# aiforvision/OCTA-autosegmentation

Measured on AMD Instinct MI355X. Metric: synthetic OCTA samples/sec (graph + 304x304 image + 1216x1216 label triples), higher is better.
Workload: dtype f64

## Files before the change

include/octa_hip.h:

```cpp
#ifndef OCTA_HIP_H
#define OCTA_HIP_H

#include <stddef.h>
#include <stdint.h>

#ifdef __cplusplus
extern "C" {
#endif

typedef struct octa_ctx octa_ctx;


int octa_abi_version(void);

const char *octa_last_error(void);

int octa_ctx_create(int device, octa_ctx **out);
void octa_ctx_destroy(octa_ctx *ctx);

size_t octa_ctx_scratch_bytes(const octa_ctx *ctx);

int octa_rasterize_2d(octa_ctx *ctx, int B, const double *d_edges, const int64_t *h_edge_off,
                      const uint8_t *d_keep, int no_pixels_x, int no_pixels_y, int mip_axis,
                      double min_radius, double max_radius, uint8_t *d_out, void *stream);
// ... 284 lines not shown
int octa_sim_geometry(int num_cus, int *h_out4);

int octa_sim_is_large(const octa_sim *sim);

int octa_sim_fields(octa_sim *sim, int sample, double *h_oxy, int64_t cap_oxy, int64_t *n_oxy, double *h_co2,
                    int64_t cap_co2, int64_t *n_co2);

int octa_sim_kat_kd_order(octa_ctx *ctx, const double *h_pts, int64_t n, const uint8_t *h_need, int32_t *h_indices);

int octa_sim_kat_kd_order_signflag(octa_ctx *ctx, const double *h_pts, int64_t n, const uint8_t *h_need, int32_t need_bits, int32_t *h_indices);

int octa_sim_kat_sample(octa_ctx *ctx, const double *h_cand, int64_t n_cand, const double *h_npos, const double *h_nrad, int64_t n_art,
                        double *h_oxy, int64_t n_oxy, int64_t cap_oxy, double eps_n, double eps_k, double eps_s, const double *h_cst8,
                        int64_t *h_n_out);

#ifdef __cplusplus
}
#endif
#endif
```

octa_autosegmentation_amd/_native.py:

```python
import contextlib
import ctypes
import os
import random as _random
import threading

import numpy as np

HERE = os.path.dirname(os.path.abspath(__file__))
LIB_PATH = os.environ.get("OCTA_HIP_LIB") or os.path.join(HERE, "liboctahip.so")

_lib = None
_ctxs = {}
_lock = threading.Lock()

c_void_p, c_int, c_double, c_size_t = ctypes.c_void_p, ctypes.c_int, ctypes.c_double, ctypes.c_size_t


def _struct(name, ints, ptrs):
    fields = [("struct_size", ctypes.c_uint32)] + [(k, c_int) for k in ints.split()] + [("slope", ctypes.c_float)] + [(k, c_void_p) for k in ptrs.split()]
    return type(name, (ctypes.Structure,), {"_fields_": fields})


Conv3x3Args = _struct("Conv3x3Args", "N H W Cin Cout stride in_dilation tap_mask out_scale out_off_y out_off_x C1 CY1 nslot",
                      "d_x d_x2 d_w d_y d_y2 d_scale1 d_shift1 d_scale2 d_shift2 d_stat_partials d_stat_slots d_residual")
# ... 113 lines not shown
    "octa_headn_nhwc_bwd": (c_int, [c_void_p, c_void_p, c_void_p, c_void_p, c_int, ctypes.c_int64, c_int, c_int, c_void_p, c_void_p, c_void_p, c_void_p]),
    "octa_conv3x3_c1_fwd": (c_int, [c_void_p, c_void_p, c_void_p, c_void_p, c_int, c_int, c_int, c_int, c_void_p, c_int, c_void_p]),
    "octa_fft2_c2c_f64_workspace_bytes": (c_size_t, [c_int, c_int, c_int]),
    "octa_fft2_c2c_f64": (c_int, [c_void_p, c_void_p, c_int, c_int, c_int, c_int, c_void_p, c_void_p]),
    "octa_oof_workspace_bytes": (c_size_t, [c_int, c_int, c_int]),
    "octa_oof_2d": (c_int, [c_void_p, c_void_p, c_int, c_int, c_int, c_void_p, c_void_p]),
    "octa_oof_2d_response": (c_int, [c_void_p, c_void_p, c_int, c_int, c_int, c_void_p, c_void_p]),
    "octa_frangi_workspace_bytes": (c_size_t, [c_int, c_int, c_int, c_int]),
    "octa_frangi_2d": (c_int, [c_void_p, c_void_p, c_int, c_int, c_int, c_int, c_void_p, c_void_p, ctypes.c_float, c_double, c_double, c_int, c_void_p, c_void_p]),
    "octa_frangi_hessian": (c_int, [c_void_p, c_void_p, c_void_p, c_void_p, c_int, c_int, c_int, c_int, c_void_p, ctypes.c_float, c_int, c_void_p, c_void_p]),
    "octa_frangi_eigenvalues": (c_int, [c_void_p, c_void_p, c_void_p, c_void_p, c_int, c_int, c_int, c_int, c_void_p, ctypes.c_float, c_int, c_void_p, c_void_p]),
    "octa_sim_kat_kd_order": (c_int, [c_void_p, c_void_p, ctypes.c_int64, c_void_p, c_void_p]),
    "octa_sim_kat_kd_order_signflag": (c_int, [c_void_p, c_void_p, ctypes.c_int64, c_void_p, ctypes.c_int32, c_void_p]),
    "octa_sim_kat_sample": (c_int, [c_void_p, c_void_p, ctypes.c_int64, c_void_p, c_void_p, ctypes.c_int64, c_void_p, ctypes.c_int64, ctypes.c_int64,
                                    c_double, c_double, c_double, c_void_p, c_void_p]),
}


class OctaHipError(RuntimeError):
    pass


def lib():
    global _lib
    if _lib is None:
        with _lock:
            if _lib is None:
                if not os.path.exists(LIB_PATH):
                    raise OctaHipError(
                        f"{LIB_PATH} is missing: build it with `python -m octa_autosegmentation_amd.build` "
# ... 113 lines not shown
```

octa_autosegmentation_amd/csrc/sim.hip:

```cpp

#include <chrono>
#include <vector>

#include "common.h"
#include "sim_host.h"
#include <thread>
#include <atomic>
#include <cstdlib>
#include <cstring>

using namespace OCTA_SIMK;

#if OCTA_SIM_LARGE
#define OCTA_SIM_T octa_simL_impl
#define OCTA_SIM_FN(name) octa_simL_##name
#else
#define OCTA_SIM_T octa_simS_impl
#define OCTA_SIM_FN(name) octa_simS_##name
#endif
#define octa_sim_create OCTA_SIM_FN(create)
#define octa_sim_destroy OCTA_SIM_FN(destroy)
#define octa_sim_run OCTA_SIM_FN(run)
#define octa_sim_run_states OCTA_SIM_FN(run_states)
#define octa_sim_np_state OCTA_SIM_FN(np_state)
#define octa_sim_edge_offsets OCTA_SIM_FN(edge_offsets)
#define octa_sim_export_edges OCTA_SIM_FN(export_edges)
#define octa_sim_export_edges_device OCTA_SIM_FN(export_edges_device)
#define octa_sim_trace OCTA_SIM_FN(trace)
#define octa_sim_stats OCTA_SIM_FN(stats)
#define octa_sim_kd_paths OCTA_SIM_FN(kd_paths)
#define octa_sim_assign_paths OCTA_SIM_FN(assign_paths)
#define octa_sim_fields OCTA_SIM_FN(fields)
#define octa_sim_service_stats OCTA_SIM_FN(service_stats)
#define octa_sim_geometry OCTA_SIM_FN(geometry)
#define octa_sim_spans OCTA_SIM_FN(spans)
#define octa_sim_timing OCTA_SIM_FN(timing)
#define octa_sim_kat_kd_order OCTA_SIM_FN(kat_kd_order)
#define octa_sim_kat_kd_order_signflag OCTA_SIM_FN(kat_kd_order_signflag)
#define octa_sim_kat_sample OCTA_SIM_FN(kat_sample)
struct OCTA_SIM_T;
extern "C" void octa_sim_destroy(OCTA_SIM_T *S);
extern "C" long long octa_sim_next_ticket(void);
extern "C" int *octa_sim_launch_flag(int device);

namespace {

constexpr int SIM_THREADS = SIM_THREADS_PER_WG;
constexpr int SIM_WG_PER_CU = 2;
#if OCTA_SIM_LARGE
constexpr size_t SIM_LDS = 2048;
#else
constexpr size_t SIM_LDS = SIM_LDS_BYTES;
static_assert((size_t)KD_MAILBOX_OFF + KD_MAILBOX_BYTES <= (size_t)SIM_USER_BYTES && SIM_WG_PER_CU * SIM_LDS <= 160 * 1024, "LDS budget");
#endif
// ... 1360 lines not shown
        ok(hipFuncSetAttribute(reinterpret_cast<const void *>(sim_kat_sample_kernel), hipFuncAttributeMaxDynamicSharedMemorySize, (int)SIM_LDS), "attribute")) {
        hipLaunchKernelGGL(sim_kat_sample_kernel, dim3(1), dim3(SIM_THREADS), SIM_LDS, 0, A, C, P);
        if (ok(hipGetLastError(), "launch") && ok(hipMemcpy(&sc, A.sc, sizeof(sc), hipMemcpyDeviceToHost), "result")) {
            if (sc.err) { octa::set_error("octa_sim_kat_sample: the phase set error bits %d", sc.err); rc = -3; }
            else {
                *h_n_out = sc.n_oxy;
                const int64_t n = sc.n_oxy < cap_oxy ? sc.n_oxy : cap_oxy;
                if (n) ok(hipMemcpy(h_oxy, A.oxy, sizeof(double) * 3 * n, hipMemcpyDeviceToHost), "sinks back");
            }
        }
    }
    (void)hipFree(d);
    return rc;
}

#endif

extern "C" int octa_sim_service_stats(OCTA_SIM_T *S, double *h_out4) {
    if (!S || !S->ran || !h_out4) { octa::set_error("octa_sim_service_stats: run the simulation first"); return -2; }
    h_out4[0] = (double)S->diag_tickets; h_out4[1] = S->diag_max_gap_ms; h_out4[2] = (double)S->diag_relaunches; h_out4[3] = (double)S->diag_parked;
    h_out4[4] = S->diag_max_bif_ms;
    return 0;
}

extern "C" int octa_sim_geometry(int num_cus, int *h_out4) {
    if (!h_out4) { octa::set_error("octa_sim_geometry: null output"); return -2; }
    h_out4[0] = SIM_THREADS; h_out4[1] = SIM_WG_PER_CU; h_out4[2] = (int)SIM_LDS; h_out4[3] = SIM_WG_PER_CU * (num_cus > 0 ? num_cus : 256);
    return 0;
}

// ... 13 lines not shown
```

octa_autosegmentation_amd/csrc/sim_api.cpp:

```cpp
#include <cstdlib>
#include <cstring>
#include <new>

#include "common.h"

extern "C" {
struct octa_simS_impl;
struct octa_simL_impl;
#define OCTA_DECL(SFX, T)                                                                                                                       \
    int octa_sim##SFX##_create(octa_ctx *, const octa_sim_config *, int, T **);                                                                 \
    void octa_sim##SFX##_destroy(T *);                                                                                                          \
    int octa_sim##SFX##_run(T *, const uint32_t *, const uint64_t *, octa_bif_fn, void *, void *);                                              \
    int octa_sim##SFX##_run_states(T *, const double *, const double *, const uint32_t *, const uint32_t *, octa_bif_fn, void *, void *);       \
    int octa_sim##SFX##_np_state(T *, int, uint32_t *);                                                                                         \
    int octa_sim##SFX##_edge_offsets(T *, int64_t *, int64_t *);                                                                                \
    int octa_sim##SFX##_export_edges(T *, double *);                                                                                            \
    int octa_sim##SFX##_export_edges_device(T *, double *, void *);                                                                             \
    int octa_sim##SFX##_trace(T *, int32_t *);                                                                                                  \
    int octa_sim##SFX##_stats(T *, int64_t *);                                                                                                  \
    int octa_sim##SFX##_kd_paths(T *, int64_t *);                                                                                               \
    int octa_sim##SFX##_assign_paths(T *, int64_t *);                                                                                           \
    int octa_sim##SFX##_spans(T *, int64_t *);                                                                                                  \
    int octa_sim##SFX##_timing(T *, double *);                                                                                                  \
    int octa_sim##SFX##_service_stats(T *, double *);                                                                                           \
    int octa_sim##SFX##_geometry(int, int *);                                                                                                   \
    int octa_sim##SFX##_fields(T *, int, double *, int64_t, int64_t *, double *, int64_t, int64_t *);
OCTA_DECL(S, octa_simS_impl)
OCTA_DECL(L, octa_simL_impl)
#undef OCTA_DECL
int octa_simS_kat_kd_order(octa_ctx *, const double *, int64_t, const uint8_t *, int32_t *);
int octa_simS_kat_kd_order_signflag(octa_ctx *, const double *, int64_t, const uint8_t *, int32_t, int32_t *);
int octa_simS_kat_sample(octa_ctx *, const double *, int64_t, const double *, const double *, int64_t, double *, int64_t, int64_t, double, double, double,
                         const double *, int64_t *);
}

#include <atomic>
#include <mutex>
static std::atomic<long long> g_sim_launches{0};
extern "C" long long octa_sim_next_ticket(void) { return g_sim_launches.fetch_add(1, std::memory_order_acq_rel) + 1; }
extern "C" long long octa_sim_launch_count(void) { return g_sim_launches.load(std::memory_order_acquire); }
extern "C" int *octa_sim_launch_flag(int device) {
    static std::mutex m;
    static int *flags[64] = {};
    if (device < 0 || device >= 64) return nullptr;
    std::lock_guard<std::mutex> g(m);
    if (!flags[device]) {
        int prev = 0;
        if (hipGetDevice(&prev) != hipSuccess || hipSetDevice(device) != hipSuccess) return nullptr;
// ... 62 lines not shown
extern "C" int octa_sim_kd_paths(octa_sim *sim, int64_t *t) { NEED(sim, "octa_sim_kd_paths") return FWD(octa_simS_kd_paths(sim->s, t), octa_simL_kd_paths(sim->l, t)); }
extern "C" int octa_sim_assign_paths(octa_sim *sim, int64_t *t) { NEED(sim, "octa_sim_assign_paths") return FWD(octa_simS_assign_paths(sim->s, t), octa_simL_assign_paths(sim->l, t)); }
extern "C" int octa_sim_spans(octa_sim *sim, int64_t *t) { NEED(sim, "octa_sim_spans") return FWD(octa_simS_spans(sim->s, t), octa_simL_spans(sim->l, t)); }
extern "C" int octa_sim_timing(octa_sim *sim, double *t) { NEED(sim, "octa_sim_timing") return FWD(octa_simS_timing(sim->s, t), octa_simL_timing(sim->l, t)); }
extern "C" int octa_sim_service_stats(octa_sim *sim, double *t) { NEED(sim, "octa_sim_service_stats") return FWD(octa_simS_service_stats(sim->s, t), octa_simL_service_stats(sim->l, t)); }
extern "C" int octa_sim_fields(octa_sim *sim, int k, double *o, int64_t co, int64_t *no, double *c, int64_t cc, int64_t *nc) {
    NEED(sim, "octa_sim_fields") return FWD(octa_simS_fields(sim->s, k, o, co, no, c, cc, nc), octa_simL_fields(sim->l, k, o, co, no, c, cc, nc));
}
extern "C" int octa_sim_geometry(int num_cus, int *h_out4) { return octa_simS_geometry(num_cus, h_out4); }
extern "C" int octa_sim_kat_kd_order(octa_ctx *ctx, const double *p, int64_t n, const uint8_t *need, int32_t *o) { return octa_simS_kat_kd_order(ctx, p, n, need, o); }
extern "C" int octa_sim_kat_kd_order_signflag(octa_ctx *ctx, const double *p, int64_t n, const uint8_t *need, int32_t bits, int32_t *o) { return octa_simS_kat_kd_order_signflag(ctx, p, n, need, bits, o); }
extern "C" int octa_sim_kat_sample(octa_ctx *ctx, const double *cand, int64_t n_cand, const double *npos, const double *nrad, int64_t n_art, double *oxy,
                                   int64_t n_oxy, int64_t cap_oxy, double eps_n, double eps_k, double eps_s, const double *cst8, int64_t *n_out) {
    return octa_simS_kat_sample(ctx, cand, n_cand, npos, nrad, n_art, oxy, n_oxy, cap_oxy, eps_n, eps_k, eps_s, cst8, n_out);
}
extern "C" int octa_sim_is_large(const octa_sim *sim) { return sim && sim->large ? 1 : 0; }
```

octa_autosegmentation_amd/csrc/sim_core.h:

```cpp
#pragma once
#include <cmath>
#include <cstdint>
#include <cstring>
#include <algorithm>
#include "gpow.h"
#include "glibc_trig.h"

#ifndef OCTA_SIM_LARGE
#define OCTA_SIM_LARGE 0
#endif
#if OCTA_SIM_LARGE
#define OCTA_SIMK octa_simk_large
#else
#define OCTA_SIMK octa_simk
#endif
namespace OCTA_SIMK {

#if OCTA_SIM_LARGE
typedef unsigned int idx_t;
typedef unsigned long long kdw_t;
constexpr int IDX_BITS = 18;
constexpr int GROUP_BITS = 17;
constexpr int NCAP = 1 << 17;
constexpr int OCAP = 1 << 18;
// ... 919 lines not shown
#if defined(__HIP_DEVICE_COMPILE__)
    atomicMin(p, v);
#else
    if (v < *p) *p = v;
#endif
}

constexpr int KD_TAB_OFF = OCAP * (int)sizeof(kdw_t);
constexpr int KD_BOX_BYTES = KD_RANGES * 24;
static_assert(KD_RANGES >= OCAP / 17 + 1, "ranges per level");
static_assert(KD_MAILBOX_OFF % 16 == 0 && KD_MAILBOX_OFF >= KD_TAB_OFF + KD_RANGES * KD_TAB_BYTES_PER_RANGE, "kd tables overlap the mailbox");
static_assert(KD_MAILBOX_OFF + (KD_BOX_BYTES > KD_MAILBOX_BYTES ? KD_BOX_BYTES : KD_MAILBOX_BYTES) <= SIM_USER_BYTES, "kd table layout (box table and mailbox share their area)");
OCTA_HD inline void kd_build(const Blk &b, const double *pts, int n, idx_t *out_idx, idx_t *out_rank,
                              float *xy, double zlo, double zhi, long *kdprof = nullptr, const unsigned char *need = nullptr,
                              const bool flag_in_sign = false, const unsigned char need_bits = 0xff) {
#if defined(__HIP_DEVICE_COMPILE__) && !defined(OCTA_SIM_PROF_ASSIGN) && !defined(OCTA_SIM_PROF_SAMPLE) && !defined(OCTA_SIM_PROF_SET) && !defined(OCTA_SIM_PROF_MAIL) && !defined(OCTA_SIM_PROF_SEQ) && !defined(OCTA_SIM_PROF_SEQ2)
#define KDP(slot) do { if (kdprof && b.tid == 0) { long _t = (long)wall_clock64(); kdprof[slot] += _t - _kt; _kt = _t; } } while (0)
    long _kt = (long)wall_clock64();
#else
#define KDP(slot) do { } while (0)
#endif
    kdw_t *kv = reinterpret_cast<kdw_t *>(b.user_of<1>());
    idx_t *tab = reinterpret_cast<idx_t *>(b.user_of<1>() + KD_TAB_OFF);
    idx_t *rs = tab, *re = tab + KD_RANGES;
    idx_t *rs2 = tab + 2 * KD_RANGES, *re2 = tab + 3 * KD_RANGES;
    signed char *rd = reinterpret_cast<signed char *>(tab + 4 * KD_RANGES);
    unsigned *bbf = reinterpret_cast<unsigned *>(b.user_of<1>() + KD_MAILBOX_OFF);
#if defined(__HIP_DEVICE_COMPILE__) && !OCTA_SIM_LARGE
    if ((size_t)n * (sizeof(kdw_t) + 8) + 8 <= (size_t)KD_TAB_OFF)
        xy = reinterpret_cast<float *>(b.user_of<1>() + (((size_t)n * sizeof(kdw_t) + 7) & ~(size_t)7));
#endif
// ... 1165 lines not shown
#else
#ifndef OCTA_SIM_SAMPLE_GRID
#define OCTA_SIM_SAMPLE_GRID 96
#endif
#ifndef OCTA_SIM_SAMPLE_NODE_FIRST
#define OCTA_SIM_SAMPLE_NODE_FIRST 0
#endif
constexpr int SMP_CH = 2048;
constexpr int SMP_GRID = OCTA_SIM_SAMPLE_GRID;
constexpr int SMP_GP_MAX = 1024, SMP_GPAIR_CAP = 2048;
constexpr size_t SMP_OFF_LIVE = (size_t)SMP_CH * 24, SMP_OFF_PP = SMP_OFF_LIVE + SMP_CH, SMP_OFF_SLOT = SMP_OFF_PP + (size_t)SMP_GP_MAX * 24;
static_assert(SMP_CH < 0xffff && SMP_GRID * SMP_GRID < 0xffff, "slots and cells are 16-bit, 0xffff marks a candidate that is not valid");
static_assert(SMP_OFF_PP + ((size_t)SMP_GRID * SMP_GRID + 2) / 2 * 4 <= SMP_OFF_SLOT && SMP_OFF_SLOT + (size_t)SMP_CH * 2 <= (size_t)SIM_USER_BYTES, "candidate grid layout");
static_assert((size_t)SMP_GP_MAX * 7 + (size_t)SMP_GPAIR_CAP * 2 <= SMP_OFF_LIVE && (size_t)ACCCAP * 24 <= SMP_OFF_PP + (size_t)SMP_GP_MAX * 24, "greedy acceptance tables");
#if defined(OCTA_SIM_SAMPLE_COUNT) && !defined(__HIP_DEVICE_COMPILE__)
static long smp_count[12];
static int smp_count_pass = 5;
#define SMP_COUNT(i, v) (smp_count[i] += (v))
#else
#define SMP_COUNT(i, v) ((void)0)
#endif
struct SmpGrid {
    int nc;
    double x0, inv;
    unsigned *endw;
    const double *pos;
    unsigned char *live;
};
OCTA_HD inline int smp_cell1(const SmpGrid &G, double x) { return grid_clampi((int)floor((x - G.x0) * G.inv), G.nc - 1); }
OCTA_HD inline int smp_end(const SmpGrid &G, int c) { return (int)((G.endw[c >> 1] >> ((c & 1) * 16)) & 0xffffu); }
template <class F>
// ... 1184 lines not shown
        sc->new_begin[f] = n_before;
        sc->new_end[f] = n_nodes;
        sc->n_nodes[f] = n_nodes;
        sc->py_pos = py_pos;
        if (b.tid == 0) {
            if (err) sc->err |= err;
            sc->murray_steps += steps + n_def;
            sc->murray_deferred += n_def;
#if defined(__HIP_DEVICE_COMPILE__)
            b.coll()[91] = n_def <= MURRAY_FLUSH_LDS ? 0 : n_def;
#else
            b.coll()[91] = n_def;
#endif
            sc->n_bif += n_bif;
            sc->respec += respec;
            sc->kdprof[7] += t_acc[0]; (void)t_acc[1]; (void)t_acc[2];
#if defined(OCTA_SIM_PROF_SEQ2) && defined(__HIP_DEVICE_COMPILE__)
            q2[3] = t_acc[1];
            for (int k = 0; k < 7; k++) sc->kdprof[k] += q2[k];
#endif
#if defined(OCTA_SIM_PROF_SEQ) && defined(__HIP_DEVICE_COMPILE__)
            sc->kdprof[1] += (long)wall_clock64() - _q1; sc->kdprof[2] += t_acc[0]; sc->kdprof[4] += t_acc[2]; sc->kdprof[5] += t_acc[3]; sc->kdprof[6] += n_def;
#endif
        }
#if defined(__HIP_DEVICE_COMPILE__)
        if (n_def > 0 && n_def <= MURRAY_FLUSH_LDS) {
            const long tp0 = (long)wall_clock64();
            for (int base = 0; base < n_def; base += MURRAY_FLUSH_WAVE)
                murray_flush_prepare_wave(A, f, L, n_def, A.fl_rec + (size_t)f * MURRAY_FLUSH_LDS, base);
            if (b.tid == 0) { sc->fl_pending[f] = n_def; sc->kdprof[7] += (long)wall_clock64() - tp0; }
        }
#endif
    }
#if defined(__HIP_DEVICE_COMPILE__)
    else {
        static_assert(SIM_THREADS_PER_WG == 256, "the ordered pass hands its side work to waves 1 - 3");
        const int wv = b.tid >> 6;
        if (wv == 1) side(side_lds);
        const int nw = (f == 1 || pend_other > 2 * MURRAY_FLUSH_WAVE) ? 3 : 2;
        const int w = wv == 2 ? 0 : (wv == 3 ? 1 : 2);
        if (w < nw && w * 64 < pend_other) {
            const int rounds = murray_flush_rounds_wave(A.nrad_of(1 - f), L.log_tab, L.exp_tab, L.fl_val, L.fl_done, A.fl_rec + (size_t)(1 - f) * MURRAY_FLUSH_LDS,
                                                        pend_other, w, nw, true);
            if (b.tid == 128) sc->flush_rounds += rounds;
        }
// ... 2 lines not shown
    (void)side; (void)side_lds;
#endif
#undef SEQT
#undef SEQ2_TOP
#undef SEQ2_SEL
#undef SEQ2_END
#undef SEQ2_ARG
    b.sync();
#if defined(__HIP_DEVICE_COMPILE__)
    if (b.tid == 0 && pend_other > 0) sc->fl_pending[1 - f] = 0;
#endif
    {
        long t0 = OCTA_FLUSH_T0();
        const int rounds = murray_flush(b, A, f, L, b.coll()[91]);
        if (b.tid == 0) {
            sc->kdprof[7] += OCTA_FLUSH_T0() - t0; sc->flush_rounds += rounds;
#if defined(OCTA_SIM_PROF_SEQ) && defined(__HIP_DEVICE_COMPILE__)
            sc->kdprof[3] += OCTA_FLUSH_T0() - t0;
#endif
        }
    }
    b.sync();
}

OCTA_HD inline void murray_flush_pending(const Blk &b, const SimArrays &A) {
#if defined(__HIP_DEVICE_COMPILE__)
    b.sync();
    double *fl_val = reinterpret_cast<double *>(b.user_of<8>());
    int *fl_done = reinterpret_cast<int *>(fl_val + MURRAY_FLUSH_LDS);
    for (int f = 0; f < 2; f++) {
        const int n = OCTA_UNI(A.sc->fl_pending[f]);
// ... 93 lines not shown
    (void)A; (void)f; (void)n;
    return false;
#else
    return OCTA_UNI((int)(A.nn_prev_of(f) != nullptr && A.sc->n_cached[f] == n)) != 0;
#endif
}

#if defined(__HIP_DEVICE_COMPILE__)
#define OCTA_SUBPROF(sc, slot, t0) do { if (b.tid == 0) { long _t1 = (long)wall_clock64(); (sc)->prof[slot] += _t1 - (t0); (t0) = _t1; } } while (0)
#define OCTA_SUBPROF_T0() ((long)wall_clock64())
#else
#define OCTA_SUBPROF(sc, slot, t0) do { (void)(t0); } while (0)
#define OCTA_SUBPROF_T0() 0L
#endif

OCTA_HD inline void phase_satisfy_art(const Blk &b, const SimArrays &A, const SimConst &C, const IterParams &P) {
    const double zext = C.sz;
    SampleScalars *sc = A.sc;
    const int nb = sc->new_begin[0], ne = sc->new_end[0];
    const int n_new = ne - nb, n_oxy = sc->n_oxy;
    if (n_new <= 0 || n_oxy <= 0) return;
    const double ek = P.eps_k, ek2 = ek * ek;
    long t0 = OCTA_SUBPROF_T0();
    for (int i = b.tid; i < n_oxy; i += b.nth) A.removed[i] = 0;
    int *ctl = b.coll() + 100;
    if (b.tid == 0) { ctl[0] = 0; ctl[1] = 0; ctl[2] = 0; }
    unsigned char *xf = reinterpret_cast<unsigned char *>(A.nn);
    static_assert((size_t)NCAP <= (size_t)OCAP * sizeof(int), "group flags fit the nearest-node list");
    for (int j = b.tid; j < n_new && j < NCAP; j += b.nth) xf[j] = 0;
    b.sync();
    {
        int *new_ids = A.tmp_int;
        for (int j = b.tid; j < n_new; j += b.nth) new_ids[j] = nb + j;
        b.sync();
        Grid G = grid_build(b, A, A.npos[0], new_ids, n_new, ek);
        for (int o = b.tid; o < n_oxy; o += b.nth) {
            const V3 p = ld3(A.oxy + 3 * o);
            grid_visit(G, p.x, p.y, ek, [&](int j, const V3 &q) {
                if (sqdist(p, q) <= ek2) {
                    int slot = atomic_add_int(&ctl[0], 1);
                    if (slot < PCAP) A.pairs[slot] = ((unsigned)(j - nb) << IDX_BITS) | (unsigned)o;
                    A.removed[o] = 1;
                }
            });
        }
        b.sync();
    }
    OCTA_SUBPROF(sc, 12, t0);
    int n_pairs = ctl[0];
    if (n_pairs > PCAP) { if (b.tid == 0) atomic_or_int(&sc->err, ERR_PAIR_CAP); n_pairs = PCAP; }
    if (n_new > (1 << (32 - IDX_BITS))) { if (b.tid == 0) atomic_or_int(&sc->err, ERR_PAIR_CAP); }
    b.sync();
    if (n_pairs == 0) return;
    {
        const int n_ven = sc->n_nodes[1];
        int *rem = A.tmp_int;
        int n_rem = 0;
        {
            const int chunk = (n_oxy + b.nth - 1) / b.nth;
            const int i0 = b.tid * chunk < n_oxy ? b.tid * chunk : n_oxy, i1 = (i0 + chunk < n_oxy) ? i0 + chunk : n_oxy;
            int local = 0;
            for (int o = i0; o < i1; o++) local += A.removed[o] ? 1 : 0;
            int ex;
            n_rem = blk_scan(b, local, &ex);
            int run = ex;
            for (int o = i0; o < i1; o++) if (A.removed[o]) rem[run++] = o;
        }
        b.sync();
        for (int k = b.tid; k < n_rem; k += b.nth) {
            const int o = rem[k];
            A.ven_near[o] = 0;
            A.hashes[o] = py_hash_tuple3(ld3(A.oxy + 3 * o));
        }
        Grid G = grid_build(b, A, A.oxy, rem, n_rem, ek);
        constexpr int VB = 4;
        for (int j0 = b.tid; j0 < n_ven; j0 += VB * b.nth) {
            V3 qv[VB];
#pragma unroll
            for (int u = 0; u < VB; u++) { const int j = j0 + u * b.nth; qv[u] = ld3(A.npos[1] + 3 * (j < n_ven ? j : n_ven - 1)); }
#pragma unroll
            for (int u = 0; u < VB; u++) {
                if (j0 + u * b.nth >= n_ven) break;
                const V3 q = qv[u];
                grid_visit(G, q.x, q.y, ek, [&](int o, const V3 &p) {
                    if (sqrt(sqdist(q, p)) <= ek) A.ven_near[o] = 1;
                });
            }
        }
        b.sync();
    }
    OCTA_SUBPROF(sc, 12, t0);
    bool set_in_lds = false;
    int rung = 0;
    bool from_partial = false;
    auto sink_of = [&](unsigned pr) -> int {
        const unsigned low = pr & IDX_MASK;
        return (rung == 2 || (rung == 1 && xf[pr >> IDX_BITS])) ? (int)A.kd_idx[low] : (int)low;
    };
#ifdef OCTA_SIM_DEBUG_SAT
    int dbg_n_ins = -1, dbg_mask = -1, dbg_base = -1;
    const int dbg_n_co2_in = sc->n_co2;
#endif
    while (true) {
        const int vslot = rung == 1 ? 2 : 1;
        if (rung > 0) {
// ... 330 lines not shown
#endif
    const bool carry = assign_memory_covers(A, 0, n_oxy);
    int keep = compact_points(b, A.oxy, n_oxy, A.removed, A.tmp_dbl, carry ? A.nn_prev[0] : nullptr, carry ? A.nn_d2[0] : nullptr);
    if (b.tid == 0) { sc->n_oxy = keep; sc->n_cached[0] = carry ? keep : 0; }
    b.sync();
    OCTA_SUBPROF(sc, 15, t0);
}

OCTA_HD inline void phase_satisfy_ven(const Blk &b, const SimArrays &A, const IterParams &P) {
    SampleScalars *sc = A.sc;
    const int nb = sc->new_begin[1], ne = sc->new_end[1];
    const int n_new = ne - nb, n_co2 = sc->n_co2;
    if (n_new <= 0 || n_co2 <= 0) return;
    const double ek2 = P.eps_k * P.eps_k;
    const double ek = P.eps_k;
    {
        int *new_ids = A.tmp_int;
        for (int j = b.tid; j < n_new; j += b.nth) new_ids[j] = nb + j;
        b.sync();
        Grid G = grid_build(b, A, A.npos[1], new_ids, n_new, ek);
        for (int o = b.tid; o < n_co2; o += b.nth) {
            const V3 p = ld3(A.co2 + 3 * o);
            bool hit = false;
            grid_visit(G, p.x, p.y, ek, [&](int, const V3 &q) {
                if (!hit && sqdist(p, q) <= ek2) hit = true;
            });
            A.removed[o] = hit ? 1 : 0;
        }
        b.sync();
    }
    const bool carry = assign_memory_covers(A, 1, n_co2);
    int keep = compact_points(b, A.co2, n_co2, A.removed, A.tmp_dbl, carry ? A.nn_prev[1] : nullptr, carry ? A.nn_d2[1] : nullptr);
    if (b.tid == 0) { sc->n_co2 = keep; sc->n_cached[1] = carry ? keep : 0; }
    b.sync();
}

}
```

Before: 1650.

## Use LDS short-list binning for satisfy phases instead of global grid

In the small simulator build, the arterial and venous satisfy phases now bin the new nodes (or removed sinks) into a shared-memory cell grid in chunks of 1024 instead of building a global-memory grid. Neighbour tests read from LDS, and the venous pass skips compaction when no source was hit. The change also adds a known-answer entry point and optional profiling and counting hooks. It is meant to cut global-memory traffic and grid build cost. In exchange it adds chunked passes when inputs exceed the chunk size and depends on the LDS layout static_asserts.

```diff
diff --git a/include/octa_hip.h b/include/octa_hip.h
--- a/include/octa_hip.h
+++ b/include/octa_hip.h
@@ -322,6 +322,10 @@
                         double *h_oxy, int64_t n_oxy, int64_t cap_oxy, double eps_n, double eps_k, double eps_s, const double *h_cst8,
                         int64_t *h_n_out);
 
+int octa_sim_kat_satisfy(octa_ctx *ctx, double *h_oxy, int64_t n_oxy, const double *h_art, int64_t n_art, int64_t nb_art, const double *h_ven,
+                         int64_t n_ven, int64_t nb_ven, double *h_co2, int64_t n_co2, int64_t cap_co2, double eps_k, double size_z,
+                         int64_t *h_out6);
+
 #ifdef __cplusplus
 }
 #endif
diff --git a/octa_autosegmentation_amd/_native.py b/octa_autosegmentation_amd/_native.py
--- a/octa_autosegmentation_amd/_native.py
+++ b/octa_autosegmentation_amd/_native.py
@@ -151,6 +151,8 @@
     "octa_sim_kat_kd_order_signflag": (c_int, [c_void_p, c_void_p, ctypes.c_int64, c_void_p, ctypes.c_int32, c_void_p]),
     "octa_sim_kat_sample": (c_int, [c_void_p, c_void_p, ctypes.c_int64, c_void_p, c_void_p, ctypes.c_int64, c_void_p, ctypes.c_int64, ctypes.c_int64,
                                     c_double, c_double, c_double, c_void_p, c_void_p]),
+    "octa_sim_kat_satisfy": (c_int, [c_void_p, c_void_p, ctypes.c_int64, c_void_p, ctypes.c_int64, ctypes.c_int64, c_void_p, ctypes.c_int64, ctypes.c_int64,
+                                     c_void_p, ctypes.c_int64, ctypes.c_int64, c_double, c_double, c_void_p]),
 }
 
 
diff --git a/octa_autosegmentation_amd/csrc/sim.hip b/octa_autosegmentation_amd/csrc/sim.hip
--- a/octa_autosegmentation_amd/csrc/sim.hip
+++ b/octa_autosegmentation_amd/csrc/sim.hip
@@ -38,6 +38,7 @@
 #define octa_sim_kat_kd_order OCTA_SIM_FN(kat_kd_order)
 #define octa_sim_kat_kd_order_signflag OCTA_SIM_FN(kat_kd_order_signflag)
 #define octa_sim_kat_sample OCTA_SIM_FN(kat_sample)
+#define octa_sim_kat_satisfy OCTA_SIM_FN(kat_satisfy)
 struct OCTA_SIM_T;
 extern "C" void octa_sim_destroy(OCTA_SIM_T *S);
 extern "C" long long octa_sim_next_ticket(void);
@@ -1428,6 +1429,81 @@
     return rc;
 }
 
+namespace {
+__global__ void __launch_bounds__(SIM_THREADS)
+sim_kat_satisfy_kernel(SimArrays A, SimConst C, IterParams P, int *n_co2_mid) {
+    extern __shared__ __attribute__((aligned(16))) unsigned char smem[];
+    Blk b = {(int)threadIdx.x, (int)blockDim.x, smem};
+    phase_satisfy_art(b, A, C, P);
+    if (b.tid == 0) *n_co2_mid = A.sc->n_co2;
+    b.sync();
+    phase_satisfy_ven(b, A, P);
+}
+}
+
+extern "C" int octa_sim_kat_satisfy(octa_ctx *ctx, double *h_oxy, int64_t n_oxy, const double *h_art, int64_t n_art, int64_t nb_art, const double *h_ven,
+                                    int64_t n_ven, int64_t nb_ven, double *h_co2, int64_t n_co2, int64_t cap_co2, double eps_k, double size_z,
+                                    int64_t *h_out6) {
+    if (!ctx || !h_out6 || n_oxy < 0 || n_oxy > OCAP || n_art < 0 || n_art > NCAP || nb_art < 0 || nb_art > n_art || n_ven < 0 || n_ven > NCAP ||
+        nb_ven < 0 || nb_ven > n_ven || n_co2 < 0 || cap_co2 < n_co2 || cap_co2 > CCAP || (n_oxy && !h_oxy) || (n_art && !h_art) || (n_ven && !h_ven) ||
+        (cap_co2 && !h_co2)) {
+        octa::set_error("octa_sim_kat_satisfy: bad arguments");
+        return -2;
+    }
+    OCTA_HIP_CHECK(hipSetDevice(ctx->device));
+    SimConst C;
+    memset(&C, 0, sizeof(C));
+    C.sz = size_z;
+    SampleScalars sc;
+    memset(&sc, 0, sizeof(sc));
+    sc.n_nodes[0] = (int)n_art; sc.n_nodes[1] = (int)n_ven; sc.n_oxy = (int)n_oxy; sc.n_co2 = (int)n_co2;
+    sc.new_begin[0] = (int)nb_art; sc.new_end[0] = (int)n_art; sc.new_begin[1] = (int)nb_ven; sc.new_end[1] = (int)n_ven;
+    IterParams P;
+    memset(&P, 0, sizeof(P));
+    P.eps_k = eps_k;
+    const size_t n_dbl = (size_t)OCAP * 3 * 2 + (size_t)CCAP * 3 + (size_t)NCAP * 3 * 2 + (size_t)GRID_N * 3, n_u64 = (size_t)OCAP + SETCAP;
+    const size_t n_int = (size_t)OCAP * 2 + 2 * (size_t)NCANDCAP + SETCAP + PCAP + 4, n_idx = (size_t)OCAP * 2, n_byte = (size_t)OCAP * 2;
+    const size_t off_u64 = n_dbl * 8, off_int = off_u64 + n_u64 * 8, off_idx = off_int + n_int * 4, off_byte = (off_idx + n_idx * sizeof(idx_t) + 15) & ~(size_t)15,
+                 off_sc = (off_byte + n_byte + 15) & ~(size_t)15;
+    unsigned char *d = nullptr;
+    OCTA_HIP_CHECK(hipMalloc(&d, off_sc + sizeof(SampleScalars)));
+    int rc = 0;
+    auto ok = [&](hipError_t e, const char *what) { if (e != hipSuccess && rc == 0) { octa::set_error("octa_sim_kat_satisfy: %s: %s", what, hipGetErrorString(e)); rc = -1; } return rc == 0; };
+    double *dd = reinterpret_cast<double *>(d);
+    SimArrays A;
+    memset((void *)&A, 0, sizeof(A));
+    A.oxy = dd; A.tmp_dbl = A.oxy + (size_t)OCAP * 3; A.co2 = A.tmp_dbl + (size_t)OCAP * 3; A.npos[0] = A.co2 + (size_t)CCAP * 3;
+    A.npos[1] = A.npos[0] + (size_t)NCAP * 3; A.grid_pts = A.npos[1] + (size_t)NCAP * 3;
+    A.hashes = reinterpret_cast<unsigned long long *>(d + off_u64); A.set_hash = A.hashes + OCAP;
+    A.nn = reinterpret_cast<int *>(d + off_int); A.tmp_int = A.nn + OCAP; A.set_key = A.tmp_int + OCAP + 2 * (size_t)NCANDCAP;
+    A.pairs = reinterpret_cast<unsigned *>(A.set_key + SETCAP);
+    int *d_mid = reinterpret_cast<int *>(A.pairs + PCAP);
+    A.kd_idx = reinterpret_cast<idx_t *>(d + off_idx); A.kd_rank = A.kd_idx + OCAP;
+    A.removed = d + off_byte; A.ven_near = A.removed + OCAP; A.sc = reinterpret_cast<SampleScalars *>(d + off_sc);
+    if (ok(hipMemset(d, 0, off_sc), "clear") && (!n_oxy || ok(hipMemcpy(A.oxy, h_oxy, sizeof(double) * 3 * n_oxy, hipMemcpyHostToDevice), "sinks")) &&
+        (!n_art || ok(hipMemcpy(A.npos[0], h_art, sizeof(double) * 3 * n_art, hipMemcpyHostToDevice), "arterial nodes")) &&
+        (!n_ven || ok(hipMemcpy(A.npos[1], h_ven, sizeof(double) * 3 * n_ven, hipMemcpyHostToDevice), "venous nodes")) &&
+        (!n_co2 || ok(hipMemcpy(A.co2, h_co2, sizeof(double) * 3 * n_co2, hipMemcpyHostToDevice), "sources")) &&
+        ok(hipMemcpy(A.sc, &sc, sizeof(sc), hipMemcpyHostToDevice), "scalars") &&
+        ok(hipFuncSetAttribute(reinterpret_cast<const void *>(sim_kat_satisfy_kernel), hipFuncAttributeMaxDynamicSharedMemorySize, (int)SIM_LDS), "attribute")) {
+        hipLaunchKernelGGL(sim_kat_satisfy_kernel, dim3(1), dim3(SIM_THREADS), SIM_LDS, 0, A, C, P, d_mid);
+        int mid = 0;
+        if (ok(hipGetLastError(), "launch") && ok(hipMemcpy(&sc, A.sc, sizeof(sc), hipMemcpyDeviceToHost), "result") &&
+            ok(hipMemcpy(&mid, d_mid, sizeof(int), hipMemcpyDeviceToHost), "count")) {
+            if (sc.err) { octa::set_error("octa_sim_kat_satisfy: a phase set error bits %d", sc.err); rc = -3; }
+            else if (sc.n_co2 > cap_co2 || mid > cap_co2) { octa::set_error("octa_sim_kat_satisfy: %d sources, room for %d", sc.n_co2 > mid ? sc.n_co2 : mid, (int)cap_co2); rc = -3; }
+            else {
+                h_out6[0] = sc.n_oxy; h_out6[1] = mid; h_out6[2] = sc.n_co2;
+                for (int k = 0; k < 3; k++) h_out6[3 + k] = sc.kd_path[k];
+                if (sc.n_oxy) ok(hipMemcpy(h_oxy, A.oxy, sizeof(double) * 3 * sc.n_oxy, hipMemcpyDeviceToHost), "sinks back");
+                if (sc.n_co2) ok(hipMemcpy(h_co2, A.co2, sizeof(double) * 3 * sc.n_co2, hipMemcpyDeviceToHost), "sources back");
+            }
+        }
+    }
+    (void)hipFree(d);
+    return rc;
+}
+
 #endif
 
 extern "C" int octa_sim_service_stats(OCTA_SIM_T *S, double *h_out4) {
diff --git a/octa_autosegmentation_amd/csrc/sim_api.cpp b/octa_autosegmentation_amd/csrc/sim_api.cpp
--- a/octa_autosegmentation_amd/csrc/sim_api.cpp
+++ b/octa_autosegmentation_amd/csrc/sim_api.cpp
@@ -32,6 +32,8 @@
 int octa_simS_kat_kd_order_signflag(octa_ctx *, const double *, int64_t, const uint8_t *, int32_t, int32_t *);
 int octa_simS_kat_sample(octa_ctx *, const double *, int64_t, const double *, const double *, int64_t, double *, int64_t, int64_t, double, double, double,
                          const double *, int64_t *);
+int octa_simS_kat_satisfy(octa_ctx *, double *, int64_t, const double *, int64_t, int64_t, const double *, int64_t, int64_t, double *, int64_t, int64_t, double,
+                          double, int64_t *);
 }
 
 #include <atomic>
@@ -124,4 +126,8 @@
                                    int64_t n_oxy, int64_t cap_oxy, double eps_n, double eps_k, double eps_s, const double *cst8, int64_t *n_out) {
     return octa_simS_kat_sample(ctx, cand, n_cand, npos, nrad, n_art, oxy, n_oxy, cap_oxy, eps_n, eps_k, eps_s, cst8, n_out);
 }
+extern "C" int octa_sim_kat_satisfy(octa_ctx *ctx, double *oxy, int64_t n_oxy, const double *art, int64_t n_art, int64_t nb_art, const double *ven, int64_t n_ven,
+                                    int64_t nb_ven, double *co2, int64_t n_co2, int64_t cap_co2, double eps_k, double size_z, int64_t *out6) {
+    return octa_simS_kat_satisfy(ctx, oxy, n_oxy, art, n_art, nb_art, ven, n_ven, nb_ven, co2, n_co2, cap_co2, eps_k, size_z, out6);
+}
 extern "C" int octa_sim_is_large(const octa_sim *sim) { return sim && sim->large ? 1 : 0; }
diff --git a/octa_autosegmentation_amd/csrc/sim_core.h b/octa_autosegmentation_amd/csrc/sim_core.h
--- a/octa_autosegmentation_amd/csrc/sim_core.h
+++ b/octa_autosegmentation_amd/csrc/sim_core.h
@@ -957,7 +957,7 @@
 OCTA_HD inline void kd_build(const Blk &b, const double *pts, int n, idx_t *out_idx, idx_t *out_rank,
                               float *xy, double zlo, double zhi, long *kdprof = nullptr, const unsigned char *need = nullptr,
                               const bool flag_in_sign = false, const unsigned char need_bits = 0xff) {
-#if defined(__HIP_DEVICE_COMPILE__) && !defined(OCTA_SIM_PROF_ASSIGN) && !defined(OCTA_SIM_PROF_SAMPLE) && !defined(OCTA_SIM_PROF_SET) && !defined(OCTA_SIM_PROF_MAIL) && !defined(OCTA_SIM_PROF_SEQ) && !defined(OCTA_SIM_PROF_SEQ2)
+#if defined(__HIP_DEVICE_COMPILE__) && !defined(OCTA_SIM_PROF_ASSIGN) && !defined(OCTA_SIM_PROF_SAMPLE) && !defined(OCTA_SIM_PROF_SET) && !defined(OCTA_SIM_PROF_MAIL) && !defined(OCTA_SIM_PROF_SEQ) && !defined(OCTA_SIM_PROF_SEQ2) && !defined(OCTA_SIM_PROF_SAT)
 #define KDP(slot) do { if (kdprof && b.tid == 0) { long _t = (long)wall_clock64(); kdprof[slot] += _t - _kt; _kt = _t; } } while (0)
     long _kt = (long)wall_clock64();
 #else
@@ -2153,7 +2153,7 @@
 static_assert(SMP_OFF_PP + ((size_t)SMP_GRID * SMP_GRID + 2) / 2 * 4 <= SMP_OFF_SLOT && SMP_OFF_SLOT + (size_t)SMP_CH * 2 <= (size_t)SIM_USER_BYTES, "candidate grid layout");
 static_assert((size_t)SMP_GP_MAX * 7 + (size_t)SMP_GPAIR_CAP * 2 <= SMP_OFF_LIVE && (size_t)ACCCAP * 24 <= SMP_OFF_PP + (size_t)SMP_GP_MAX * 24, "greedy acceptance tables");
 #if defined(OCTA_SIM_SAMPLE_COUNT) && !defined(__HIP_DEVICE_COMPILE__)
-static long smp_count[12];
+static long smp_count[14];
 static int smp_count_pass = 5;
 #define SMP_COUNT(i, v) (smp_count[i] += (v))
 #else
@@ -3368,7 +3368,10 @@
 #endif
             sc->n_bif += n_bif;
             sc->respec += respec;
-            sc->kdprof[7] += t_acc[0]; (void)t_acc[1]; (void)t_acc[2];
+#ifndef OCTA_SIM_PROF_SAT
+            sc->kdprof[7] += t_acc[0];
+#endif
+            (void)t_acc[0]; (void)t_acc[1]; (void)t_acc[2];
 #if defined(OCTA_SIM_PROF_SEQ2) && defined(__HIP_DEVICE_COMPILE__)
             q2[3] = t_acc[1];
             for (int k = 0; k < 7; k++) sc->kdprof[k] += q2[k];
@@ -3382,7 +3385,13 @@
             const long tp0 = (long)wall_clock64();
             for (int base = 0; base < n_def; base += MURRAY_FLUSH_WAVE)
                 murray_flush_prepare_wave(A, f, L, n_def, A.fl_rec + (size_t)f * MURRAY_FLUSH_LDS, base);
-            if (b.tid == 0) { sc->fl_pending[f] = n_def; sc->kdprof[7] += (long)wall_clock64() - tp0; }
+            if (b.tid == 0) {
+                sc->fl_pending[f] = n_def;
+#ifndef OCTA_SIM_PROF_SAT
+                sc->kdprof[7] += (long)wall_clock64() - tp0;
+#endif
+                (void)tp0;
+            }
         }
 #endif
     }
@@ -3415,7 +3424,11 @@
         long t0 = OCTA_FLUSH_T0();
         const int rounds = murray_flush(b, A, f, L, b.coll()[91]);
         if (b.tid == 0) {
-            sc->kdprof[7] += OCTA_FLUSH_T0() - t0; sc->flush_rounds += rounds;
+#ifndef OCTA_SIM_PROF_SAT
+            sc->kdprof[7] += OCTA_FLUSH_T0() - t0;
+#endif
+            (void)t0;
+            sc->flush_rounds += rounds;
 #if defined(OCTA_SIM_PROF_SEQ) && defined(__HIP_DEVICE_COMPILE__)
             sc->kdprof[3] += OCTA_FLUSH_T0() - t0;
 #endif
@@ -3539,6 +3552,89 @@
 #define OCTA_SUBPROF_T0() 0L
 #endif
 
+#if (OCTA_SIM_LARGE || defined(OCTA_SIM_SAMPLE_DIRECT)) && !defined(OCTA_SIM_SATISFY_GRID)
+#define OCTA_SIM_SATISFY_GRID
+#endif
+#ifndef OCTA_SIM_SATISFY_GRID
+constexpr int SL_CH = 1024;
+constexpr size_t SL_OFF_LIVE = (size_t)SL_CH * 24, SL_OFF_ID = SL_OFF_LIVE + SL_CH, SL_OFF_END = SL_OFF_ID + (size_t)SL_CH * 4,
+                 SL_OFF_CELL = SL_OFF_END + ((size_t)SMP_GRID * SMP_GRID + 2) / 2 * 4;
+static_assert(SL_CH < 0xffff && SL_OFF_END % 4 == 0 && SL_OFF_CELL + (size_t)SL_CH * 2 <= (size_t)SIM_USER_BYTES, "short-list layout");
+struct ShortList {
+    SmpGrid G;
+    int *id;
+};
+OCTA_HD inline ShortList shortlist_bin(const Blk &b, const double *pts, const int *ids, int first, int n, double radius) {
+    unsigned char *const U = b.user_of<2>();
+    ShortList S;
+    SmpGrid &G = S.G;
+    double *const pos = reinterpret_cast<double *>(U);
+    unsigned short *const cell_of = reinterpret_cast<unsigned short *>(U + SL_OFF_CELL);
+    S.id = reinterpret_cast<int *>(U + SL_OFF_ID);
+    {
+        const double cell = fmax(radius, 1.2 / SMP_GRID);
+        const int nc = (int)ceil(1.2 / cell);
+        G.nc = nc < 1 ? 1 : (nc > SMP_GRID ? SMP_GRID : nc);
+        G.x0 = -0.1; G.inv = 1.0 / cell; G.endw = reinterpret_cast<unsigned *>(U + SL_OFF_END); G.pos = pos; G.live = U + SL_OFF_LIVE;
+    }
+    const int nc = G.nc, nwords = (nc * nc + 2) / 2;
+    b.sync();
+    for (int w = b.tid; w < nwords; w += b.nth) G.endw[w] = 0;
+    b.sync();
+    for (int i = b.tid; i < n; i += b.nth) {
+        const double *p = pts + 3 * (size_t)(ids ? ids[i] : first + i);
+        const int c = smp_cell1(G, p[1]) * nc + smp_cell1(G, p[0]);
+        atomic_add_int(reinterpret_cast<int *>(&G.endw[c >> 1]), 1 << ((c & 1) * 16));
+        cell_of[i] = (unsigned short)c;
+    }
+    b.sync();
+    {
+        const int chunk = ((nwords + b.nth - 1) / b.nth) | 1;
+        const int w0 = b.tid * chunk < nwords ? b.tid * chunk : nwords, w1 = w0 + chunk < nwords ? w0 + chunk : nwords;
+        int local = 0;
+        for (int w = w0; w < w1; w++) { const unsigned v = G.endw[w]; local += (int)(v & 0xffffu) + (int)(v >> 16); }
+        int ex;
+        blk_scan(b, local, &ex);
+        unsigned run = (unsigned)ex;
+        for (int w = w0; w < w1; w++) {
+            const unsigned v = G.endw[w], lo = v & 0xffffu, hi = v >> 16;
+            G.endw[w] = run | ((run + lo) << 16);
+            run += lo + hi;
+        }
+    }
+    b.sync();
+    for (int i = b.tid; i < n; i += b.nth) {
+        const int c = cell_of[i], sh = (c & 1) * 16;
+        const V3 p = ld3(pts + 3 * (size_t)(ids ? ids[i] : first + i));
+        const int k = (int)(((unsigned)atomic_add_int(reinterpret_cast<int *>(&G.endw[c >> 1]), 1 << sh) >> sh) & 0xffffu);
+        st3(pos + 3 * k, p);
+        G.live[k] = 1;
+        S.id[k] = i;
+    }
+    b.sync();
+    return S;
+}
+constexpr double SL_PAD = 1e-9;
+#if defined(OCTA_SIM_SAMPLE_COUNT) && !defined(__HIP_DEVICE_COMPILE__)
+#define SL_COUNT_PASS() (smp_count_pass = 12)
+#else
+#define SL_COUNT_PASS() ((void)0)
+#endif
+#endif
+
+#if defined(OCTA_SIM_PROF_SAT) && defined(__HIP_DEVICE_COMPILE__)
+#define SATP_T0() long _qt = (long)wall_clock64()
+#define SATP(slot) do { b.sync(); if (b.tid == 0) { long _t = (long)wall_clock64(); sc->kdprof[slot] += _t - _qt; _qt = _t; } } while (0)
+#else
+#define SATP_T0() do { } while (0)
+#define SATP(slot) do { } while (0)
+#endif
+#if defined(OCTA_SIM_SAT_COUNT) && !defined(__HIP_DEVICE_COMPILE__)
+static long sat_count[10];
+#define SAT_COUNT(i, v) (sat_count[i] += (v))
+#else
+#define SAT_COUNT(i, v) ((void)0)
+#endif
 OCTA_HD inline void phase_satisfy_art(const Blk &b, const SimArrays &A, const SimConst &C, const IterParams &P) {
     const double zext = C.sz;
     SampleScalars *sc = A.sc;
@@ -3547,6 +3643,7 @@
     if (n_new <= 0 || n_oxy <= 0) return;
     const double ek = P.eps_k, ek2 = ek * ek;
     long t0 = OCTA_SUBPROF_T0();
+    SAT_COUNT(0, 1); SAT_COUNT(1, n_new); SAT_COUNT(2, n_oxy);
     for (int i = b.tid; i < n_oxy; i += b.nth) A.removed[i] = 0;
     int *ctl = b.coll() + 100;
     if (b.tid == 0) { ctl[0] = 0; ctl[1] = 0; ctl[2] = 0; }
@@ -3554,11 +3651,14 @@
     static_assert((size_t)NCAP <= (size_t)OCAP * sizeof(int), "group flags fit the nearest-node list");
     for (int j = b.tid; j < n_new && j < NCAP; j += b.nth) xf[j] = 0;
     b.sync();
+    SATP_T0();
+#ifdef OCTA_SIM_SATISFY_GRID
     {
         int *new_ids = A.tmp_int;
         for (int j = b.tid; j < n_new; j += b.nth) new_ids[j] = nb + j;
         b.sync();
         Grid G = grid_build(b, A, A.npos[0], new_ids, n_new, ek);
+        SATP(0);
         for (int o = b.tid; o < n_oxy; o += b.nth) {
             const V3 p = ld3(A.oxy + 3 * o);
             grid_visit(G, p.x, p.y, ek, [&](int j, const V3 &q) {
@@ -3570,13 +3670,50 @@
             });
         }
         b.sync();
-    }
+        SATP(1);
+    }
+#else
+    int *const rem = A.tmp_int;
+    if (b.tid == 0) ctl[3] = 0;
+    SL_COUNT_PASS();
+    for (int c0 = 0; c0 < n_new; c0 += SL_CH) {
+        const ShortList S = shortlist_bin(b, A.npos[0], nullptr, nb + c0, n_new - c0 < SL_CH ? n_new - c0 : SL_CH, ek);
+        SATP(0);
+        constexpr int SB = 4;
+        for (int i0 = b.tid; i0 < n_oxy; i0 += SB * b.nth) {
+            V3 s[SB];
+#pragma unroll
+            for (int u = 0; u < SB; u++) { const int i = i0 + u * b.nth; s[u] = ld3(A.oxy + 3 * (size_t)(i < n_oxy ? i : n_oxy - 1)); }
+            OCTA_ISSUE_LOADS();
+#pragma unroll
+            for (int u = 0; u < SB; u++) {
+                const int o = i0 + u * b.nth;
+                if (o >= n_oxy) break;
+                const V3 p = s[u];
+                bool first = true;
+                smp_visit(S.G, p.x, p.y, ek + SL_PAD, [&](int k, const V3 &q) {
+                    if (sqdist(p, q) <= ek2) {
+                        const int slot = atomic_add_int(&ctl[0], 1);
+                        if (slot < PCAP) A.pairs[slot] = ((unsigned)(c0 + S.id[k]) << IDX_BITS) | (unsigned)o;
+                        if (first) {
+                            first = false;
+                            if (!A.removed[o]) { A.removed[o] = 1; rem[atomic_add_int(&ctl[3], 1)] = o; }
+                        }
+                    }
+                });
+            }
+        }
+        SATP(1);
+    }
+    b.sync();
+#endif
     OCTA_SUBPROF(sc, 12, t0);
     int n_pairs = ctl[0];
     if (n_pairs > PCAP) { if (b.tid == 0) atomic_or_int(&sc->err, ERR_PAIR_CAP); n_pairs = PCAP; }
     if (n_new > (1 << (32 - IDX_BITS))) { if (b.tid == 0) atomic_or_int(&sc->err, ERR_PAIR_CAP); }
     b.sync();
     if (n_pairs == 0) return;
+#ifdef OCTA_SIM_SATISFY_GRID
     {
         const int n_ven = sc->n_nodes[1];
         int *rem = A.tmp_int;
@@ -3597,7 +3734,9 @@
             A.ven_near[o] = 0;
             A.hashes[o] = py_hash_tuple3(ld3(A.oxy + 3 * o));
         }
+        SATP(2); SAT_COUNT(3, 1); SAT_COUNT(4, n_rem); SAT_COUNT(5, n_ven);
         Grid G = grid_build(b, A, A.oxy, rem, n_rem, ek);
+        SATP(3);
         constexpr int VB = 4;
         for (int j0 = b.tid; j0 < n_ven; j0 += VB * b.nth) {
             V3 qv[VB];
@@ -3613,7 +3752,45 @@
             }
         }
         b.sync();
-    }
+        SATP(4);
+    }
+#else
+    {
+        const int n_ven = sc->n_nodes[1];
+        const int n_rem = OCTA_UNI(ctl[3]);
+        const double ek_sq = sqrt_le_bound(ek);
+        SAT_COUNT(3, 1); SAT_COUNT(4, n_rem); SAT_COUNT(5, n_ven);
+        for (int c0 = 0; c0 < n_rem; c0 += SL_CH) {
+            const int n = n_rem - c0 < SL_CH ? n_rem - c0 : SL_CH;
+            const ShortList S = shortlist_bin(b, A.oxy, rem + c0, 0, n, ek);
+            SATP(3);
+            constexpr int VB = 4;
+            for (int j0 = b.tid; j0 < n_ven; j0 += VB * b.nth) {
+                V3 qv[VB];
+#pragma unroll
+                for (int u = 0; u < VB; u++) { const int j = j0 + u * b.nth; qv[u] = ld3(A.npos[1] + 3 * (size_t)(j < n_ven ? j : n_ven - 1)); }
+                OCTA_ISSUE_LOADS();
+#pragma unroll
+                for (int u = 0; u < VB; u++) {
+                    if (j0 + u * b.nth >= n_ven) break;
+                    const V3 q = qv[u];
+                    smp_visit(S.G, q.x, q.y, ek + SL_PAD, [&](int k, const V3 &p) {
+                        if (sqdist(q, p) <= ek_sq) S.G.live[k] = 0;
+                    });
+                }
+            }
+            b.sync();
+            SATP(4);
+            for (int k = b.tid; k < n; k += b.nth) {
+                const int o = rem[c0 + S.id[k]];
+                A.ven_near[o] = S.G.live[k] ? 0 : 1;
+                A.hashes[o] = py_hash_tuple3(ld3(S.G.pos + 3 * k));
+            }
+            SATP(2);
+        }
+        b.sync();
+    }
+#endif
     OCTA_SUBPROF(sc, 12, t0);
     bool set_in_lds = false;
     int rung = 0;
@@ -3974,11 +4151,15 @@
     if (n_new <= 0 || n_co2 <= 0) return;
     const double ek2 = P.eps_k * P.eps_k;
     const double ek = P.eps_k;
+    SAT_COUNT(6, 1); SAT_COUNT(7, n_new); SAT_COUNT(8, n_co2);
+    SATP_T0();
+#ifdef OCTA_SIM_SATISFY_GRID
     {
         int *new_ids = A.tmp_int;
         for (int j = b.tid; j < n_new; j += b.nth) new_ids[j] = nb + j;
         b.sync();
         Grid G = grid_build(b, A, A.npos[1], new_ids, n_new, ek);
+        SATP(5);
         for (int o = b.tid; o < n_co2; o += b.nth) {
             const V3 p = ld3(A.co2 + 3 * o);
             bool hit = false;
@@ -3988,11 +4169,59 @@
             A.removed[o] = hit ? 1 : 0;
         }
         b.sync();
+        SATP(6);
     }
     const bool carry = assign_memory_covers(A, 1, n_co2);
     int keep = compact_points(b, A.co2, n_co2, A.removed, A.tmp_dbl, carry ? A.nn_prev[1] : nullptr, carry ? A.nn_d2[1] : nullptr);
     if (b.tid == 0) { sc->n_co2 = keep; sc->n_cached[1] = carry ? keep : 0; }
     b.sync();
-}
-
-}
+    SATP(7); SAT_COUNT(9, keep == n_co2);
+#else
+    int *ctl = b.coll() + 100;
+    if (b.tid == 0) ctl[0] = 0;
+    SL_COUNT_PASS();
+    for (int c0 = 0; c0 < n_new; c0 += SL_CH) {
+        const ShortList S = shortlist_bin(b, A.npos[1], nullptr, nb + c0, n_new - c0 < SL_CH ? n_new - c0 : SL_CH, ek);
+        SATP(5);
+        constexpr int SB = 4;
+        bool any = false;
+        for (int i0 = b.tid; i0 < n_co2; i0 += SB * b.nth) {
+            V3 s[SB];
+#pragma unroll
+            for (int u = 0; u < SB; u++) { const int i = i0 + u * b.nth; s[u] = ld3(A.co2 + 3 * (size_t)(i < n_co2 ? i : n_co2 - 1)); }
+            OCTA_ISSUE_LOADS();
+#pragma unroll
+            for (int u = 0; u < SB; u++) {
+                const int o = i0 + u * b.nth;
+                if (o >= n_co2) break;
+                const V3 p = s[u];
+                bool hit = false;
+                smp_visit(S.G, p.x, p.y, ek + SL_PAD, [&](int, const V3 &q) {
+                    if (!hit && sqdist(p, q) <= ek2) hit = true;
+                });
+                if (c0 == 0) A.removed[o] = hit ? 1 : 0;
+                else if (hit) A.removed[o] = 1;
+                any |= hit;
+            }
+        }
+        if (any) atomic_or_int(&ctl[0], 1);
+        SATP(6);
+    }
+    b.sync();
+    const bool none = ctl[0] == 0;
+    const bool carry = assign_memory_covers(A, 1, n_co2);
+    b.sync();
+    if (none) {
+        if (b.tid == 0) sc->n_cached[1] = carry ? n_co2 : 0;
+        b.sync();
+        SATP(7); SAT_COUNT(9, 1);
+        return;
+    }
+    int keep = compact_points(b, A.co2, n_co2, A.removed, A.tmp_dbl, carry ? A.nn_prev[1] : nullptr, carry ? A.nn_d2[1] : nullptr);
+    if (b.tid == 0) { sc->n_co2 = keep; sc->n_cached[1] = carry ? keep : 0; }
+    b.sync();
+    SATP(7); SAT_COUNT(9, keep == n_co2);
+#endif
+}
+
+}
```

New measurement: 1693, median of 6. +2.6%, better.
